# PeterFWS/Structure-PLP-SLAM

Measured on NVIDIA H100. Metric: frames_per_sec_extract_match_poseopt, higher is better.
Workload: dtype u8/f64

## Files before the change

structure-plp-slam_b200/csrc/orb.cu:

```cuda
#include "common.cuh"
#include <cuda.h>
#include <stdlib.h>
#include "brief_pattern.inc"
#include "quadtree_kernels.cuh"

namespace plp {

namespace {

constexpr int kMaxLevels = 16;
constexpr int kHalfPatch = 15;
constexpr int kCellSize = 64;
constexpr int kOverlap = 6;

struct LevelInfo {
    int w, h, pitch;
    size_t offset;
    size_t blur_offset;
    int cells_x, cells_y;
    int cell_base;
    int num_cells;
    int budget;
    int slot_base;
    int slot_cap;
    float scale_factor;
    float size;
};

struct CellDesc {
    short level, i, j, pad;
    short min_x, min_y, max_x, max_y;
};

struct BlurTile {
    short level, x0, y0, pad;
};

struct OrbDev {
    int num_levels, rows, cols;
    int num_cells;
    int total_slots;
    int out_cap;
    int ini_thr, min_thr;
    LevelInfo lv[kMaxLevels];
    int u_max[16];
    const uint8_t *img0;
    size_t img0_step, img0_frame_stride;
    const uint8_t *mask;
    size_t mask_step;
    uint8_t *pyr;
    size_t pyr_frame_bytes;
    uint8_t *blur;
    size_t blur_frame_bytes;
    const BlurTile *blur_tiles;
    int num_blur_tiles;
    const CellDesc *cells;
    uint32_t *cell_buf;
    int *cell_cnt;
    LevelKp *lvl_kp;
    int *lvl_cnt;
    uint8_t *qt_scratch;
    size_t qt_scratch_per_job;
    int *status;
};

__device__ __forceinline__ const uint8_t *level_ptr(const OrbDev &P, int b, int l) {
    return l == 0 ? P.img0 + (size_t)b * P.img0_frame_stride : P.pyr + (size_t)b * P.pyr_frame_bytes + P.lv[l].offset;
}
__device__ __forceinline__ int level_pitch(const OrbDev &P, int l) { return l == 0 ? (int)P.img0_step : P.lv[l].pitch; }

constexpr int kBtW = 64, kBtH = 32;
constexpr int kBoxW = 96, kBoxH = kBtH + 6, kBoxX = 16;
static_assert(kBoxW >= kBoxX + kBtW + 3 && kBoxW % 16 == 0 && kBoxX % 16 == 0 && kBtW % 16 == 0,
              "TMA box: 16-byte aligned start and extent covering the 3-pixel halo");
static_assert(kBoxH % 2 == 0 && kBtH % 2 == 0, "the blur passes work on pairs of rows");
constexpr int kBoxStage = (kBoxH * kBoxW + 127) & ~127;
constexpr int kTilePitch = kBoxW;
constexpr int kTileRows = kCellSize + kOverlap;

struct BlurMaps {
    CUtensorMap m[kMaxLevels];
};

__device__ __forceinline__ uint32_t smem_u32(const void *p) { return (uint32_t)__cvta_generic_to_shared(p); }

__device__ __forceinline__ void mbar_init(uint32_t bar) { asm volatile("mbarrier.init.shared::cta.b64 [%0], 1;" ::"r"(bar)); }

__device__ __forceinline__ bool mbar_wait(uint32_t bar, uint32_t parity) {
    uint32_t done = 0;
    for (int spin = 0; spin < (1 << 14) && !done; ++spin)
        asm volatile(
// ... 3 lines not shown
            : "memory");
    return done != 0;
}

__device__ __forceinline__ void mbar_expect_tx(uint32_t bar, uint32_t bytes) {
    asm volatile("mbarrier.arrive.expect_tx.shared::cta.b64 _, [%0], %1;" ::"r"(bar), "r"(bytes) : "memory");
}

__device__ __forceinline__ void tma_box_load(uint32_t dst, const CUtensorMap *tm, int x, int y, int f, uint32_t bar) {
    asm volatile(
        "cp.async.bulk.tensor.3d.shared::cluster.global.mbarrier::complete_tx::bytes [%0], [%1, {%2, %3, %4}], [%5];"
        ::"r"(dst), "l"(tm), "r"(x), "r"(y), "r"(f), "r"(bar)
        : "memory");
}

constexpr int kResizeRows = 8;
__global__ void __launch_bounds__(256) pyr_resize_kernel(OrbDev P, int l, const short4 *__restrict__ xtab,
                                                         const short4 *__restrict__ ytab) {
    const int b = blockIdx.y;
    const int dw = P.lv[l].w, dh = P.lv[l].h, dpitch = P.lv[l].pitch;
    const int quads = (dw + 3) >> 2, strips = (dh + kResizeRows - 1) / kResizeRows;
    const int q = blockIdx.x * blockDim.x + threadIdx.x;
    if (q >= quads * strips) return;
    const int strip = q / quads, x0 = (q - strip * quads) * 4;
    const uint8_t *src = level_ptr(P, b, l - 1);
    const int spitch = level_pitch(P, l - 1);
    uint8_t *dst = const_cast<uint8_t *>(level_ptr(P, b, l));
    int sx0[4], sx1[4], a0[4], a1[4];
#pragma unroll
    for (int k = 0; k < 4; ++k) {
        const short4 xt = xtab[min(x0 + k, dw - 1)];
        sx0[k] = xt.x;
        sx1[k] = xt.y;
        a0[k] = xt.z;
        a1[k] = xt.w;
    }
    const int y_end = min(dh, (strip + 1) * kResizeRows);
    for (int y = strip * kResizeRows; y < y_end; ++y) {
        const short4 yt = ytab[y];
        const uint8_t *S0 = src + (size_t)yt.x * spitch, *S1 = src + (size_t)yt.y * spitch;
        const int b0 = yt.z, b1 = yt.w;
        uint32_t packed = 0;
#pragma unroll
        for (int k = 0; k < 4; ++k) {
            const int r0 = S0[sx0[k]] * a0[k] + S0[sx1[k]] * a1[k];
            const int r1 = S1[sx0[k]] * a0[k] + S1[sx1[k]] * a1[k];
            const int v = (((b0 * (r0 >> 4)) >> 16) + ((b1 * (r1 >> 4)) >> 16) + 2) >> 2;
            packed |= (uint32_t)(v & 0xff) << (8 * k);
        }
        *reinterpret_cast<uint32_t *>(dst + (size_t)y * dpitch + x0) = packed;
    }
}

__device__ __forceinline__ uint32_t fast_m_pair(const uint8_t *pa, const uint8_t *pb) {
    const uint32_t v2 = ((uint32_t)pa[0] + 256u) | (((uint32_t)pb[0] + 256u) << 16);
    uint32_t d[16];
#define PLP_RING(k, off) d[k] = v2 - ((uint32_t)pa[off] | ((uint32_t)pb[off] << 16))
    PLP_RING(0, 3 * kTilePitch);
    PLP_RING(1, 3 * kTilePitch + 1);
    PLP_RING(2, 2 * kTilePitch + 2);
    PLP_RING(3, 1 * kTilePitch + 3);
    PLP_RING(4, 3);
    PLP_RING(5, -1 * kTilePitch + 3);
    PLP_RING(6, -2 * kTilePitch + 2);
    PLP_RING(7, -3 * kTilePitch + 1);
// ... 296 lines not shown
    }
    __syncthreads();
    if (n > 0) fast_cell_emit(P, b, first + n - 1, S);
}

constexpr int kDescWarps = 4;
constexpr int kDescRun = 8;
constexpr int kDescMinBlocks = 5;
constexpr int kDiscRows = 2 * kHalfPatch + 1, kDiscPitch = 48;
constexpr int kWinHalf = 18, kWinRows = 2 * kWinHalf + 1, kWinPitch = 64;
constexpr int kDiscBytes = kDiscRows * kDiscPitch;
constexpr int kDescStage = kDiscBytes + kWinRows * kWinPitch;
static_assert(kDiscBytes % 16 == 0 && kDescStage % 16 == 0, "16-byte copies into every row of the ring");
static_assert(15 + kDiscRows <= kDiscPitch && 15 + kWinRows <= kWinPitch, "the aligned supersets fit the rows");

__device__ __forceinline__ int reflect101(int p, int len) {
    if (p < 0) p = -p;
    if (p >= len) p = 2 * (len - 1) - p;
    return p;
}

__device__ __forceinline__ float fast_atan2_deg(float y, float x) {
    const float scale = (float)(180.0 / 3.14159265358979323846);
    const float p1 = 0.9997878412794807f * scale, p3 = -0.3258083974640975f * scale,
                p5 = 0.1555786518463281f * scale, p7 = -0.04432655554792128f * scale;
    const float ax = fabsf(x), ay = fabsf(y);
    float a, c, c2;
    if (ax >= ay) {
        c = __fdiv_rn(ay, ax + (float)2.2204460492503131e-16);
        c2 = c * c;
        a = (((p7 * c2 + p5) * c2 + p3) * c2 + p1) * c;
    } else {
        c = __fdiv_rn(ax, ay + (float)2.2204460492503131e-16);
        c2 = c * c;
        a = 90.f - (((p7 * c2 + p5) * c2 + p3) * c2 + p1) * c;
    }
// ... 8 lines not shown
    return c1 + v2 * (c2 + c3 * v2);
}
__device__ __forceinline__ float util_cos(float v) {
    const float PI = 3.14159265358979f, PI_2 = PI / 2.0f, TWO_PI = 2.0f * PI, INV_TWO_PI = 1.0f / TWO_PI,
                THREE_PI_2 = 3.0f * PI_2;
    v = v - (float)cv_floor((double)(v * INV_TWO_PI)) * TWO_PI;
    v = (0.0f < v) ? v : -v;
    if (v < PI_2) return poly_cos(v);
    if (v < PI) return -poly_cos(PI - v);
    if (v < THREE_PI_2) return -poly_cos(v - PI);
    return poly_cos(TWO_PI - v);
}
__device__ __forceinline__ float util_sin(float v) {
    const float PI_2 = 3.14159265358979f / 2.0f;
    return util_cos(PI_2 - v);
}


__device__ __forceinline__ void blur_row4(const uint32_t *w, uint32_t h[4]) {
    const uint32_t A = w[0], B = w[1], C = w[2];
    const uint32_t kW1 = 0x38302212u, kW2 = 0x00122230u;
    h[0] = __dp4a(__funnelshift_r(A, B, 8), kW1, __dp4a(__funnelshift_r(B, C, 8), kW2, 0u));
    h[1] = __dp4a(__funnelshift_r(A, B, 16), kW1, __dp4a(__funnelshift_r(B, C, 16), kW2, 0u));
    h[2] = __dp4a(__funnelshift_r(A, B, 24), kW1, __dp4a(__funnelshift_r(B, C, 24), kW2, 0u));
    h[3] = __dp4a(B, kW1, __dp4a(C, kW2, 0u));
}
__device__ __forceinline__ void blur_h_pass(const uint8_t *box, uint32_t *h2) {
    const uint32_t *src32 = reinterpret_cast<const uint32_t *>(box);
    for (int i = threadIdx.x; i < (kBoxH / 2) * (kBtW / 4); i += blockDim.x) {
        const int rp = i / (kBtW / 4), j = i % (kBtW / 4);
        const uint32_t *w = src32 + 2 * rp * (kBoxW / 4) + j + (kBoxX - 4) / 4;
        uint32_t e[4], o[4];
        blur_row4(w, e);
        blur_row4(w + kBoxW / 4, o);
        *reinterpret_cast<uint4 *>(h2 + rp * kBtW + 4 * j) =
            make_uint4(__byte_perm(e[0], o[0], 0x5410), __byte_perm(e[1], o[1], 0x5410), __byte_perm(e[2], o[2], 0x5410),
                       __byte_perm(e[3], o[3], 0x5410));
    }
}

constexpr int kBlurThreads = 256;
static_assert((kBtH / 2) * (kBtW / 4) == kBlurThreads, "one vertical-pass job per thread");
__device__ __forceinline__ void blur_v_pass(const uint32_t *h2, uint8_t *dst, int dpitch, int x0, int y0, int W, int H) {
    const int q = threadIdx.x / (kBtW / 4), px = (threadIdx.x % (kBtW / 4)) * 4;
    const int y = y0 + 2 * q;
    if (y >= H || x0 + px >= W) return;
    uint32_t r[4][4];
#pragma unroll
    for (int k = 0; k < 4; ++k) {
        const uint4 v = *reinterpret_cast<const uint4 *>(h2 + (q + k) * kBtW + px);
        r[k][0] = v.x;
        r[k][1] = v.y;
        r[k][2] = v.z;
        r[k][3] = v.w;
    }
    auto row = [&](uint32_t k0, uint32_t k1, uint32_t k2, uint32_t k3) -> uint32_t {
        uint32_t a[4];
#pragma unroll
        for (int c = 0; c < 4; ++c)
            a[c] = __dp2a_lo(r[0][c], k0, __dp2a_lo(r[1][c], k1, __dp2a_lo(r[2][c], k2, __dp2a_lo(r[3][c], k3, 32768u))));
        return __byte_perm(__byte_perm(a[0], a[1], 0x0062), __byte_perm(a[2], a[3], 0x0062), 0x5410);
    };
    uint8_t *d = dst + (size_t)y * dpitch + x0 + px;
    *reinterpret_cast<uint32_t *>(d) = row(0x2212u, 0x3830u, 0x2230u, 0x0012u);
    if (y + 1 < H) *reinterpret_cast<uint32_t *>(d + dpitch) = row(0x1200u, 0x3022u, 0x3038u, 0x1222u);
}

__global__ void __launch_bounds__(kBlurThreads) blur_tiles_kernel(OrbDev P) {
    __shared__ __align__(16) uint8_t s_src[kBoxH * kBoxW];
    __shared__ __align__(16) uint32_t s_h2[(kBoxH / 2) * kBtW];
    const int b = blockIdx.y, tid = threadIdx.x;
    const BlurTile t = P.blur_tiles[blockIdx.x];
    const int l = t.level, W = P.lv[l].w, H = P.lv[l].h;
    const uint8_t *img = level_ptr(P, b, l);
    const int pitch = level_pitch(P, l);
    constexpr int kCols = kBtW + 8;
    for (int i = tid; i < kBoxH * kCols; i += kBlurThreads) {
        const int py = i / kCols, px = i - py * kCols;
        const int gy = reflect101(min(t.y0 - 3 + py, H + 2), H);
        const int gx = reflect101(min(max(t.x0 - 4 + px, -3), W + 2), W);
        s_src[py * kBoxW + kBoxX - 4 + px] = img[(size_t)gy * pitch + gx];
    }
    __syncthreads();
    blur_h_pass(s_src, s_h2);
    __syncthreads();
    blur_v_pass(s_h2, P.blur + (size_t)b * P.blur_frame_bytes + P.lv[l].blur_offset, P.lv[l].pitch, t.x0, t.y0, W, H);
}

__device__ void blur_reflect_box(uint8_t *box, int bx0, int by0, int W, int H) {
    for (int i = threadIdx.x; i < kBoxH * 6; i += blockDim.x) {
        const int py = i / 6, k = i - py * 6;
        const int gx = k < 3 ? k - 3 : W + (k - 3), gy = by0 + py;
        const int px = gx - bx0;
        if (gy < 0 || gy >= H || px < 0 || px >= kBoxW) continue;
        box[py * kBoxW + px] = box[py * kBoxW + (reflect101(gx, W) - bx0)];
    }
    __syncthreads();
    for (int i = threadIdx.x; i < 6 * kBoxW; i += blockDim.x) {
        const int k = i / kBoxW, px = i - k * kBoxW;
        const int gy = k < 3 ? k - 3 : H + (k - 3);
        const int py = gy - by0;
        if (py < 0 || py >= kBoxH) continue;
        box[py * kBoxW + px] = box[(reflect101(gy, H) - by0) * kBoxW + px];
    }
    __syncthreads();
}

constexpr int kBlurRun = 4;
__global__ void __launch_bounds__(kBlurThreads) blur_tiles_tma_kernel(const __grid_constant__ BlurMaps M, OrbDev P, int run) {
    __shared__ __align__(128) uint8_t s_src[2][kBoxStage];
    __shared__ __align__(16) uint32_t s_h2[(kBoxH / 2) * kBtW];
    __shared__ __align__(8) unsigned long long s_bar[2];
    const int b = blockIdx.y, tid = threadIdx.x;
    const int first = blockIdx.x * run, n = min(run, P.num_blur_tiles - first);
    if (tid == 0) {
        mbar_init(smem_u32(&s_bar[0]));
        mbar_init(smem_u32(&s_bar[1]));
        asm volatile("fence.mbarrier_init.release.cluster;" ::: "memory");
    }
    __syncthreads();
    auto issue = [&](int i) {
        const BlurTile t = P.blur_tiles[first + i];
        const uint32_t bar = smem_u32(&s_bar[i & 1]);
        mbar_expect_tx(bar, kBoxH * kBoxW);
        tma_box_load(smem_u32(s_src[i & 1]), &M.m[t.level], t.x0 - kBoxX, t.y0 - 3, b, bar);
    };
    if (tid == 0) issue(0);
    for (int i = 0; i < n; ++i) {
        __syncthreads();
        if (tid == 0 && i + 1 < n) {
            asm volatile("fence.proxy.async.shared::cta;" ::: "memory");
            issue(i + 1);
        }
        const BlurTile t = P.blur_tiles[first + i];
        const int l = t.level, W = P.lv[l].w, H = P.lv[l].h;
        const int bx0 = t.x0 - kBoxX, by0 = t.y0 - 3;
        uint8_t *box = s_src[i & 1];
        if (!mbar_wait(smem_u32(&s_bar[i & 1]), (i >> 1) & 1)) P.status[b] = 3;
        if (t.x0 < 3 || by0 < 0 || t.x0 + kBtW + 3 > W || by0 + kBoxH > H) blur_reflect_box(box, bx0, by0, W, H);
        blur_h_pass(box, s_h2);
        __syncthreads();
        blur_v_pass(s_h2, P.blur + (size_t)b * P.blur_frame_bytes + P.lv[l].blur_offset, P.lv[l].pitch, t.x0, t.y0, W, H);
    }
}

__device__ __forceinline__ void cp_async16(void *dst, const void *src) {
    asm volatile("cp.async.ca.shared.global [%0], [%1], 16;" ::"r"(smem_u32(dst)), "l"(src) : "memory");
}
__device__ __forceinline__ void cp_async_commit() { asm volatile("cp.async.commit_group;" ::: "memory"); }
__device__ __forceinline__ void cp_async_wait_prev() { asm volatile("cp.async.wait_group 1;" ::: "memory"); }

__device__ __forceinline__ int dp4a_us(uint32_t a, uint32_t b, int c) {
    int d;
    asm("dp4a.u32.s32 %0, %1, %2, %3;" : "=r"(d) : "r"(a), "r"(b), "r"(c));
    return d;
}

template <int J>
// ... 197 lines not shown
    J.scratch_per_job = D.qt_scratch_per_job;
    J.status = D.status;
    return J;
}

struct plp_orb {
    plp_ctx *ctx = nullptr;
    plp_orb_params params;
    int rows = 0, cols = 0, max_batch = 0;
    OrbDev dev;
    std::vector<float> scale_factors, inv_scale_factors, level_sigma_sq, inv_level_sigma_sq;
    std::vector<uint32_t> num_keypts_per_level;
    std::vector<CellDesc> cells;
    short4 *d_xtab[kMaxLevels] = {nullptr};
    short4 *d_ytab[kMaxLevels] = {nullptr};
    CellDesc *d_cells = nullptr;
    uint8_t *d_pyr = nullptr;
    uint8_t *d_blur = nullptr;
    BlurTile *d_blur_tiles = nullptr;
    std::vector<BlurTile> blur_tiles;
    uint8_t *d_img = nullptr;
    uint8_t *d_mask = nullptr;
    uint32_t *d_cell_buf = nullptr;
    int *d_cell_cnt = nullptr;
    LevelKp *d_lvl_kp = nullptr;
    int *d_lvl_cnt = nullptr;
    uint8_t *d_qt_scratch = nullptr;
    int *d_status = nullptr;
    plp_keypoint *d_kp = nullptr;
    uint8_t *d_desc = nullptr;
// ... 22 lines not shown
            return nullptr;
        return (EncodeTiledFn)p;
    }();
    return fn;
}
static bool encode_level_map(CUtensorMap *m, const uint8_t *base, int w, int h, int frames, size_t pitch, size_t frame_stride) {
    EncodeTiledFn enc = tensor_map_encoder();
    if (!enc || ((uintptr_t)base & 15) || (pitch & 15) || (frame_stride & 15) || w < 1 || h < 1 || frames < 1) return false;
    const cuuint64_t dims[3] = {(cuuint64_t)w, (cuuint64_t)h, (cuuint64_t)frames};
    const cuuint64_t strides[2] = {(cuuint64_t)pitch, (cuuint64_t)frame_stride};
    const cuuint32_t box[3] = {(cuuint32_t)kBoxW, (cuuint32_t)kBoxH, 1u}, estr[3] = {1u, 1u, 1u};
    return enc(m, CU_TENSOR_MAP_DATA_TYPE_UINT8, 3, (void *)base, dims, strides, box, estr, CU_TENSOR_MAP_INTERLEAVE_NONE,
               CU_TENSOR_MAP_SWIZZLE_NONE, CU_TENSOR_MAP_L2_PROMOTION_L2_128B, CU_TENSOR_MAP_FLOAT_OOB_FILL_NONE) == CUDA_SUCCESS;
}


static void build_resize_tables(int sw, int sh, int dw, int dh, std::vector<short4> &xt, std::vector<short4> &yt) {
    const double inv_scale_x = (double)dw / sw, inv_scale_y = (double)dh / sh;
    const double scale_x = 1. / inv_scale_x, scale_y = 1. / inv_scale_y;
    xt.resize(dw);
    yt.resize(dh);
    for (int dx = 0; dx < dw; ++dx) {
        float fx = (float)((dx + 0.5) * scale_x - 0.5);
        int sx = cv_floor(fx);
        fx -= sx;
        if (sx < 0) {
            fx = 0;
            sx = 0;
        }
        if (sx >= sw - 1) {
            fx = 0;
            sx = sw - 1;
        }
        short4 t;
        t.x = (short)sx;
        t.y = (short)std::min(sx + 1, sw - 1);
        t.z = (short)lrintf((1.f - fx) * 2048);
        t.w = (short)lrintf(fx * 2048);
        xt[dx] = t;
    }
    for (int dy = 0; dy < dh; ++dy) {
        float fy = (float)((dy + 0.5) * scale_y - 0.5);
        int sy = cv_floor(fy);
        fy -= sy;
        short4 t;
        t.x = (short)std::min(std::max(sy, 0), sh - 1);
        t.y = (short)std::min(std::max(sy + 1, 0), sh - 1);
        t.z = (short)lrintf((1.f - fy) * 2048);
        t.w = (short)lrintf(fy * 2048);
        yt[dy] = t;
    }
}

extern "C" {

void plp_orb_destroy(plp_orb *o) {
    if (!o) return;
    cudaSetDevice(o->ctx->device);
    cudaStreamSynchronize(o->ctx->stream);
    for (int l = 0; l < kMaxLevels; ++l) {
        if (o->d_xtab[l]) cudaFree(o->d_xtab[l]);
        if (o->d_ytab[l]) cudaFree(o->d_ytab[l]);
    }
    void *ptrs[] = {o->d_blur, o->d_blur_tiles, o->d_cells, o->d_pyr, o->d_img, o->d_mask, o->d_cell_buf, o->d_cell_cnt, o->d_lvl_kp,
                    o->d_lvl_cnt, o->d_qt_scratch, o->d_status, o->d_kp, o->d_desc, o->d_n};
    for (void *p : ptrs)
        if (p) cudaFree(p);
// ... 73 lines not shown
        if (l == 0) {
            V.w = cols;
            V.h = rows;
        } else {
            const double scale = o->scale_factors[l];
            V.w = (int)std::round(cols * 1.0 / scale);
            V.h = (int)std::round(rows * 1.0 / scale);
        }
        V.pitch = (V.w + 63) & ~63;
        V.offset = pyr_bytes;
        if (l > 0) pyr_bytes += (size_t)V.pitch * V.h + 256;
        pyr_bytes = (pyr_bytes + 255) & ~(size_t)255;
        V.blur_offset = blur_bytes;
        blur_bytes += (size_t)V.pitch * V.h + 256;
        blur_bytes = (blur_bytes + 255) & ~(size_t)255;
        for (int y0 = 0; y0 < V.h; y0 += kBtH)
            for (int x0 = 0; x0 < V.w; x0 += kBtW) o->blur_tiles.push_back(BlurTile{(short)l, (short)x0, (short)y0, 0});
        V.budget = (int)o->num_keypts_per_level[l];
        V.scale_factor = o->scale_factors[l];
        V.size = (float)(unsigned)(31 * o->scale_factors[l]);
        V.slot_base = slot_base;
        {
            int g0 = 1;
            if (V.w > 2 * kPatchRadius && V.h > 2 * kPatchRadius) {
                const double ratio = (double)(V.w - 2 * kPatchRadius) / (V.h - 2 * kPatchRadius);
                g0 = ratio > 1 ? (int)std::round(ratio) : (int)std::round(1 / ratio);
            }
            V.slot_cap = 4 * std::max(V.budget, g0) + 8;
        }
        slot_base += V.slot_cap;
        V.cell_base = cell_base;
        V.num_cells = 0;
// ... 37 lines not shown
        qt_max_cells = std::max(qt_max_cells, V.num_cells);
    }
    if (st == PLP_OK && qt_max_cells + 1 > 2 * (qt_max_slots <= kNodeCapSmall ? kNodeCapSmall : kNodeCap)) {
        set_error("orb: a pyramid level of %d FAST cells exceeds the quadtree's cell capacity", qt_max_cells);
        st = PLP_ERR_CAPACITY;
    }
    if (st != PLP_OK) {
        delete o;
        return st;
    }
    D.num_cells = cell_base;
    D.total_slots = slot_base;
    D.out_cap = slot_base;
    D.pyr_frame_bytes = pyr_bytes ? pyr_bytes : 256;
    D.blur_frame_bytes = blur_bytes ? blur_bytes : 256;
    D.num_blur_tiles = (int)o->blur_tiles.size();
    const size_t B = (size_t)max_batch;
#define ORB_ALLOC(ptr, bytes)                                              \
    do {                                                                   \
        cudaError_t e_ = cudaMalloc((void **)&(ptr), (bytes) ? (bytes) : 256); \
        if (e_ != cudaSuccess) {                                           \
            set_error("orb: cudaMalloc(%zu) failed: %s", (size_t)(bytes), cudaGetErrorString(e_)); \
            plp_orb_destroy(o);                                            \
            return PLP_ERR_CUDA;                                           \
        }                                                                  \
    } while (0)
    for (unsigned l = 1; l < L; ++l) {
        std::vector<short4> xt, yt;
        build_resize_tables(D.lv[l - 1].w, D.lv[l - 1].h, D.lv[l].w, D.lv[l].h, xt, yt);
        ORB_ALLOC(o->d_xtab[l], xt.size() * sizeof(short4));
        ORB_ALLOC(o->d_ytab[l], yt.size() * sizeof(short4));
        cudaMemcpy(o->d_xtab[l], xt.data(), xt.size() * sizeof(short4), cudaMemcpyHostToDevice);
        cudaMemcpy(o->d_ytab[l], yt.data(), yt.size() * sizeof(short4), cudaMemcpyHostToDevice);
    }
    ORB_ALLOC(o->d_cells, o->cells.size() * sizeof(CellDesc));
    if (!o->cells.empty())
        cudaMemcpy(o->d_cells, o->cells.data(), o->cells.size() * sizeof(CellDesc), cudaMemcpyHostToDevice);
    ORB_ALLOC(o->d_pyr, B * D.pyr_frame_bytes);
    ORB_ALLOC(o->d_blur, B * D.blur_frame_bytes);
    ORB_ALLOC(o->d_blur_tiles, o->blur_tiles.size() * sizeof(BlurTile));
    if (!o->blur_tiles.empty())
        cudaMemcpy(o->d_blur_tiles, o->blur_tiles.data(), o->blur_tiles.size() * sizeof(BlurTile), cudaMemcpyHostToDevice);
    ORB_ALLOC(o->d_img, B * (size_t)rows * cols);
    ORB_ALLOC(o->d_mask, (size_t)rows * cols);
// ... 56 lines not shown

static plp_status orb_run(plp_orb *o, const uint8_t *d_imgs, int batch, size_t step, const uint8_t *d_mask,
                          size_t mask_step, plp_keypoint *d_kp, uint8_t *d_desc, int32_t *d_n, int32_t *d_status) {
    plp_ctx *ctx = o->ctx;
    OrbDev D = o->dev;
    D.img0 = d_imgs;
    D.img0_step = step;
    D.img0_frame_stride = step * (size_t)o->rows;
    D.mask = d_mask;
    D.mask_step = mask_step;
    D.status = d_status ? d_status : o->d_status;
    o->last_batch = batch;
    o->last_img0 = d_imgs;
    o->last_step = step;
    PLP_CUDA_TRY(cudaMemsetAsync(D.status, 0, (size_t)batch * sizeof(int), ctx->stream));
    for (int l = 1; l < D.num_levels; ++l) {
        const int quads = ((D.lv[l].w + 3) >> 2) * ((D.lv[l].h + kResizeRows - 1) / kResizeRows);
        if (quads <= 0) continue;
        dim3 grid(div_up(quads, 256), batch);
        PLP_LAUNCH(ctx, pyr_resize_kernel, grid, 256, 0, D, l, o->d_xtab[l], o->d_ytab[l]);
    }
    bool tma = o->maps_ok;
    if (tma && (o->map0_img != d_imgs || o->map0_step != step || o->map0_batch != batch)) {
        tma = encode_level_map(&o->maps.m[0], d_imgs, D.lv[0].w, D.lv[0].h, batch, step, D.img0_frame_stride);
        o->map0_img = tma ? d_imgs : nullptr;
        o->map0_step = step;
        o->map0_batch = batch;
    }
    if (D.num_cells > 0) {
        dim3 grid(D.num_cells, batch), grid_run(div_up(D.num_cells, kFastRun), batch);
        if (tma)
            PLP_LAUNCH(ctx, fast_cells_tma_kernel, grid_run, 256, 0, o->maps, D, kFastRun);
        else
            PLP_LAUNCH(ctx, fast_cells_kernel_v2, grid, 256, 0, D);
    }
    if (D.num_blur_tiles > 0) {
        dim3 grid(D.num_blur_tiles, batch), grid_run(div_up(D.num_blur_tiles, kBlurRun), batch);
        if (tma)
            PLP_LAUNCH(ctx, blur_tiles_tma_kernel, grid_run, kBlurThreads, 0, o->maps, D, kBlurRun);
        else
            PLP_LAUNCH(ctx, blur_tiles_kernel, grid, kBlurThreads, 0, D);
    }
    {
        dim3 grid(D.num_levels, batch);
        if (ctx->timing) plp::timing_begin(ctx, o->qt_small ? "quadtree_kernel<1024>" : "quadtree_kernel<2048>");
        const QtJob J = qt_job(D);
        if (o->qt_small)
            kQtSmall<<<grid, kQtThreadsSmall, o->qt_smem, ctx->stream>>>(J);
        else
            kQtLarge<<<grid, kQtThreadsLarge, o->qt_smem, ctx->stream>>>(J);
        if (ctx->timing) plp::timing_end(ctx);
        ctx->launches++;
    }
    {
        const int kp_est = std::max(256, (int)o->params.max_num_keypts);
        dim3 grid(div_up(std::min(D.total_slots, kp_est), kDescWarps * kDescRun), batch);
// ... 132 lines not shown
```

Before: 93160.

## Fuse pyramid resize into per-level blur tile kernel using TMA-loaded boxes

Removes the standalone pyramid resize kernels and computes each next pyramid level from the shared-memory source box already loaded for blurring, launching blur+resize per level in sequence. This avoids re-reading each level from global memory for the resize and removes separate launches. In exchange, levels must be processed serially (blur of level l produces level l+1 before its blur), adding dependency chains and host-side validation that bilinear taps fit within tile boxes.

```diff
diff --git a/structure-plp-slam_b200/csrc/orb.cu b/structure-plp-slam_b200/csrc/orb.cu
--- a/structure-plp-slam_b200/csrc/orb.cu
+++ b/structure-plp-slam_b200/csrc/orb.cu
@@ -3,6 +3,7 @@
 #include <stdlib.h>
 #include "brief_pattern.inc"
 #include "quadtree_kernels.cuh"
+#include "pyramid_kernels.cuh"
 
 namespace plp {
 
@@ -20,6 +21,8 @@
     int cells_x, cells_y;
     int cell_base;
     int num_cells;
+    int tile_base;
+    int num_tiles;
     int budget;
     int slot_base;
     int slot_cap;
@@ -30,10 +33,6 @@
 struct CellDesc {
     short level, i, j, pad;
     short min_x, min_y, max_x, max_y;
-};
-
-struct BlurTile {
-    short level, x0, y0, pad;
 };
 
 struct OrbDev {
@@ -53,7 +52,6 @@
     uint8_t *blur;
     size_t blur_frame_bytes;
     const BlurTile *blur_tiles;
-    int num_blur_tiles;
     const CellDesc *cells;
     uint32_t *cell_buf;
     int *cell_cnt;
@@ -69,12 +67,6 @@
 }
 __device__ __forceinline__ int level_pitch(const OrbDev &P, int l) { return l == 0 ? (int)P.img0_step : P.lv[l].pitch; }
 
-constexpr int kBtW = 64, kBtH = 32;
-constexpr int kBoxW = 96, kBoxH = kBtH + 6, kBoxX = 16;
-static_assert(kBoxW >= kBoxX + kBtW + 3 && kBoxW % 16 == 0 && kBoxX % 16 == 0 && kBtW % 16 == 0,
-              "TMA box: 16-byte aligned start and extent covering the 3-pixel halo");
-static_assert(kBoxH % 2 == 0 && kBtH % 2 == 0, "the blur passes work on pairs of rows");
-constexpr int kBoxStage = (kBoxH * kBoxW + 127) & ~127;
 constexpr int kTilePitch = kBoxW;
 constexpr int kTileRows = kCellSize + kOverlap;
 
@@ -108,41 +100,43 @@
         : "memory");
 }
 
-constexpr int kResizeRows = 8;
-__global__ void __launch_bounds__(256) pyr_resize_kernel(OrbDev P, int l, const short4 *__restrict__ xtab,
-                                                         const short4 *__restrict__ ytab) {
-    const int b = blockIdx.y;
-    const int dw = P.lv[l].w, dh = P.lv[l].h, dpitch = P.lv[l].pitch;
-    const int quads = (dw + 3) >> 2, strips = (dh + kResizeRows - 1) / kResizeRows;
-    const int q = blockIdx.x * blockDim.x + threadIdx.x;
-    if (q >= quads * strips) return;
-    const int strip = q / quads, x0 = (q - strip * quads) * 4;
-    const uint8_t *src = level_ptr(P, b, l - 1);
-    const int spitch = level_pitch(P, l - 1);
-    uint8_t *dst = const_cast<uint8_t *>(level_ptr(P, b, l));
-    int sx0[4], sx1[4], a0[4], a1[4];
-#pragma unroll
-    for (int k = 0; k < 4; ++k) {
-        const short4 xt = xtab[min(x0 + k, dw - 1)];
-        sx0[k] = xt.x;
-        sx1[k] = xt.y;
-        a0[k] = xt.z;
-        a1[k] = xt.w;
-    }
-    const int y_end = min(dh, (strip + 1) * kResizeRows);
-    for (int y = strip * kResizeRows; y < y_end; ++y) {
-        const short4 yt = ytab[y];
-        const uint8_t *S0 = src + (size_t)yt.x * spitch, *S1 = src + (size_t)yt.y * spitch;
-        const int b0 = yt.z, b1 = yt.w;
-        uint32_t packed = 0;
-#pragma unroll
-        for (int k = 0; k < 4; ++k) {
-            const int r0 = S0[sx0[k]] * a0[k] + S0[sx1[k]] * a1[k];
-            const int r1 = S1[sx0[k]] * a0[k] + S1[sx1[k]] * a1[k];
-            const int v = (((b0 * (r0 >> 4)) >> 16) + ((b1 * (r1 >> 4)) >> 16) + 2) >> 2;
-            packed |= (uint32_t)(v & 0xff) << (8 * k);
-        }
-        *reinterpret_cast<uint32_t *>(dst + (size_t)y * dpitch + x0) = packed;
+constexpr int kBlurRun = 4;
+constexpr int kBlurMinBlocks = 8;
+__global__ void __launch_bounds__(kBlurThreads, kBlurMinBlocks) blur_tiles_tma_kernel(const __grid_constant__ BlurMaps M, PyrJob J, int run) {
+    __shared__ __align__(128) uint8_t s_src[2][kBoxStage];
+    __shared__ __align__(16) uint32_t s_h2[(kBoxH / 2) * kBtW];
+    __shared__ __align__(8) unsigned long long s_bar[2];
+    const int b = blockIdx.y, tid = threadIdx.x;
+    const int first = blockIdx.x * run, n = min(run, J.num_tiles - first);
+    const int W = J.w, H = J.h;
+    if (tid == 0) {
+        mbar_init(smem_u32(&s_bar[0]));
+        mbar_init(smem_u32(&s_bar[1]));
+        asm volatile("fence.mbarrier_init.release.cluster;" ::: "memory");
+    }
+    __syncthreads();
+    auto issue = [&](int i) {
+        const BlurTile t = J.tiles[first + i];
+        const uint32_t bar = smem_u32(&s_bar[i & 1]);
+        mbar_expect_tx(bar, kBoxH * kBoxW);
+        tma_box_load(smem_u32(s_src[i & 1]), &M.m[t.level], t.x0 - kBoxX, t.y0 - 3, b, bar);
+    };
+    if (tid == 0) issue(0);
+    for (int i = 0; i < n; ++i) {
+        __syncthreads();
+        if (tid == 0 && i + 1 < n) {
+            asm volatile("fence.proxy.async.shared::cta;" ::: "memory");
+            issue(i + 1);
+        }
+        const BlurTile t = J.tiles[first + i];
+        const int bx0 = t.x0 - kBoxX, by0 = t.y0 - 3;
+        uint8_t *box = s_src[i & 1];
+        if (!mbar_wait(smem_u32(&s_bar[i & 1]), (i >> 1) & 1)) J.status[b] = 3;
+        if (t.x0 < 3 || by0 < 0 || t.x0 + kBtW + 3 > W || by0 + kBoxH > H) blur_reflect_box(box, bx0, by0, W, H);
+        blur_h_pass(box, s_h2);
+        if (J.dst) pyr_resize_tile(box, bx0, by0, t, J, b);
+        __syncthreads();
+        blur_v_pass(s_h2, J.blur + (size_t)b * J.blur_frame, J.blur_pitch, t.x0, t.y0, W, H);
     }
 }
 
@@ -469,12 +463,6 @@
 static_assert(kDiscBytes % 16 == 0 && kDescStage % 16 == 0, "16-byte copies into every row of the ring");
 static_assert(15 + kDiscRows <= kDiscPitch && 15 + kWinRows <= kWinPitch, "the aligned supersets fit the rows");
 
-__device__ __forceinline__ int reflect101(int p, int len) {
-    if (p < 0) p = -p;
-    if (p >= len) p = 2 * (len - 1) - p;
-    return p;
-}
-
 __device__ __forceinline__ float fast_atan2_deg(float y, float x) {
     const float scale = (float)(180.0 / 3.14159265358979323846);
     const float p1 = 0.9997878412794807f * scale, p3 = -0.3258083974640975f * scale,
@@ -513,134 +501,6 @@
 __device__ __forceinline__ float util_sin(float v) {
     const float PI_2 = 3.14159265358979f / 2.0f;
     return util_cos(PI_2 - v);
-}
-
-
-__device__ __forceinline__ void blur_row4(const uint32_t *w, uint32_t h[4]) {
-    const uint32_t A = w[0], B = w[1], C = w[2];
-    const uint32_t kW1 = 0x38302212u, kW2 = 0x00122230u;
-    h[0] = __dp4a(__funnelshift_r(A, B, 8), kW1, __dp4a(__funnelshift_r(B, C, 8), kW2, 0u));
-    h[1] = __dp4a(__funnelshift_r(A, B, 16), kW1, __dp4a(__funnelshift_r(B, C, 16), kW2, 0u));
-    h[2] = __dp4a(__funnelshift_r(A, B, 24), kW1, __dp4a(__funnelshift_r(B, C, 24), kW2, 0u));
-    h[3] = __dp4a(B, kW1, __dp4a(C, kW2, 0u));
-}
-__device__ __forceinline__ void blur_h_pass(const uint8_t *box, uint32_t *h2) {
-    const uint32_t *src32 = reinterpret_cast<const uint32_t *>(box);
-    for (int i = threadIdx.x; i < (kBoxH / 2) * (kBtW / 4); i += blockDim.x) {
-        const int rp = i / (kBtW / 4), j = i % (kBtW / 4);
-        const uint32_t *w = src32 + 2 * rp * (kBoxW / 4) + j + (kBoxX - 4) / 4;
-        uint32_t e[4], o[4];
-        blur_row4(w, e);
-        blur_row4(w + kBoxW / 4, o);
-        *reinterpret_cast<uint4 *>(h2 + rp * kBtW + 4 * j) =
-            make_uint4(__byte_perm(e[0], o[0], 0x5410), __byte_perm(e[1], o[1], 0x5410), __byte_perm(e[2], o[2], 0x5410),
-                       __byte_perm(e[3], o[3], 0x5410));
-    }
-}
-
-constexpr int kBlurThreads = 256;
-static_assert((kBtH / 2) * (kBtW / 4) == kBlurThreads, "one vertical-pass job per thread");
-__device__ __forceinline__ void blur_v_pass(const uint32_t *h2, uint8_t *dst, int dpitch, int x0, int y0, int W, int H) {
-    const int q = threadIdx.x / (kBtW / 4), px = (threadIdx.x % (kBtW / 4)) * 4;
-    const int y = y0 + 2 * q;
-    if (y >= H || x0 + px >= W) return;
-    uint32_t r[4][4];
-#pragma unroll
-    for (int k = 0; k < 4; ++k) {
-        const uint4 v = *reinterpret_cast<const uint4 *>(h2 + (q + k) * kBtW + px);
-        r[k][0] = v.x;
-        r[k][1] = v.y;
-        r[k][2] = v.z;
-        r[k][3] = v.w;
-    }
-    auto row = [&](uint32_t k0, uint32_t k1, uint32_t k2, uint32_t k3) -> uint32_t {
-        uint32_t a[4];
-#pragma unroll
-        for (int c = 0; c < 4; ++c)
-            a[c] = __dp2a_lo(r[0][c], k0, __dp2a_lo(r[1][c], k1, __dp2a_lo(r[2][c], k2, __dp2a_lo(r[3][c], k3, 32768u))));
-        return __byte_perm(__byte_perm(a[0], a[1], 0x0062), __byte_perm(a[2], a[3], 0x0062), 0x5410);
-    };
-    uint8_t *d = dst + (size_t)y * dpitch + x0 + px;
-    *reinterpret_cast<uint32_t *>(d) = row(0x2212u, 0x3830u, 0x2230u, 0x0012u);
-    if (y + 1 < H) *reinterpret_cast<uint32_t *>(d + dpitch) = row(0x1200u, 0x3022u, 0x3038u, 0x1222u);
-}
-
-__global__ void __launch_bounds__(kBlurThreads) blur_tiles_kernel(OrbDev P) {
-    __shared__ __align__(16) uint8_t s_src[kBoxH * kBoxW];
-    __shared__ __align__(16) uint32_t s_h2[(kBoxH / 2) * kBtW];
-    const int b = blockIdx.y, tid = threadIdx.x;
-    const BlurTile t = P.blur_tiles[blockIdx.x];
-    const int l = t.level, W = P.lv[l].w, H = P.lv[l].h;
-    const uint8_t *img = level_ptr(P, b, l);
-    const int pitch = level_pitch(P, l);
-    constexpr int kCols = kBtW + 8;
-    for (int i = tid; i < kBoxH * kCols; i += kBlurThreads) {
-        const int py = i / kCols, px = i - py * kCols;
-        const int gy = reflect101(min(t.y0 - 3 + py, H + 2), H);
-        const int gx = reflect101(min(max(t.x0 - 4 + px, -3), W + 2), W);
-        s_src[py * kBoxW + kBoxX - 4 + px] = img[(size_t)gy * pitch + gx];
-    }
-    __syncthreads();
-    blur_h_pass(s_src, s_h2);
-    __syncthreads();
-    blur_v_pass(s_h2, P.blur + (size_t)b * P.blur_frame_bytes + P.lv[l].blur_offset, P.lv[l].pitch, t.x0, t.y0, W, H);
-}
-
-__device__ void blur_reflect_box(uint8_t *box, int bx0, int by0, int W, int H) {
-    for (int i = threadIdx.x; i < kBoxH * 6; i += blockDim.x) {
-        const int py = i / 6, k = i - py * 6;
-        const int gx = k < 3 ? k - 3 : W + (k - 3), gy = by0 + py;
-        const int px = gx - bx0;
-        if (gy < 0 || gy >= H || px < 0 || px >= kBoxW) continue;
-        box[py * kBoxW + px] = box[py * kBoxW + (reflect101(gx, W) - bx0)];
-    }
-    __syncthreads();
-    for (int i = threadIdx.x; i < 6 * kBoxW; i += blockDim.x) {
-        const int k = i / kBoxW, px = i - k * kBoxW;
-        const int gy = k < 3 ? k - 3 : H + (k - 3);
-        const int py = gy - by0;
-        if (py < 0 || py >= kBoxH) continue;
-        box[py * kBoxW + px] = box[(reflect101(gy, H) - by0) * kBoxW + px];
-    }
-    __syncthreads();
-}
-
-constexpr int kBlurRun = 4;
-__global__ void __launch_bounds__(kBlurThreads) blur_tiles_tma_kernel(const __grid_constant__ BlurMaps M, OrbDev P, int run) {
-    __shared__ __align__(128) uint8_t s_src[2][kBoxStage];
-    __shared__ __align__(16) uint32_t s_h2[(kBoxH / 2) * kBtW];
-    __shared__ __align__(8) unsigned long long s_bar[2];
-    const int b = blockIdx.y, tid = threadIdx.x;
-    const int first = blockIdx.x * run, n = min(run, P.num_blur_tiles - first);
-    if (tid == 0) {
-        mbar_init(smem_u32(&s_bar[0]));
-        mbar_init(smem_u32(&s_bar[1]));
-        asm volatile("fence.mbarrier_init.release.cluster;" ::: "memory");
-    }
-    __syncthreads();
-    auto issue = [&](int i) {
-        const BlurTile t = P.blur_tiles[first + i];
-        const uint32_t bar = smem_u32(&s_bar[i & 1]);
-        mbar_expect_tx(bar, kBoxH * kBoxW);
-        tma_box_load(smem_u32(s_src[i & 1]), &M.m[t.level], t.x0 - kBoxX, t.y0 - 3, b, bar);
-    };
-    if (tid == 0) issue(0);
-    for (int i = 0; i < n; ++i) {
-        __syncthreads();
-        if (tid == 0 && i + 1 < n) {
-            asm volatile("fence.proxy.async.shared::cta;" ::: "memory");
-            issue(i + 1);
-        }
-        const BlurTile t = P.blur_tiles[first + i];
-        const int l = t.level, W = P.lv[l].w, H = P.lv[l].h;
-        const int bx0 = t.x0 - kBoxX, by0 = t.y0 - 3;
-        uint8_t *box = s_src[i & 1];
-        if (!mbar_wait(smem_u32(&s_bar[i & 1]), (i >> 1) & 1)) P.status[b] = 3;
-        if (t.x0 < 3 || by0 < 0 || t.x0 + kBtW + 3 > W || by0 + kBoxH > H) blur_reflect_box(box, bx0, by0, W, H);
-        blur_h_pass(box, s_h2);
-        __syncthreads();
-        blur_v_pass(s_h2, P.blur + (size_t)b * P.blur_frame_bytes + P.lv[l].blur_offset, P.lv[l].pitch, t.x0, t.y0, W, H);
-    }
 }
 
 __device__ __forceinline__ void cp_async16(void *dst, const void *src) {
@@ -868,6 +728,7 @@
     std::vector<CellDesc> cells;
     short4 *d_xtab[kMaxLevels] = {nullptr};
     short4 *d_ytab[kMaxLevels] = {nullptr};
+    int tap_words[kMaxLevels] = {0};
     CellDesc *d_cells = nullptr;
     uint8_t *d_pyr = nullptr;
     uint8_t *d_blur = nullptr;
@@ -920,43 +781,6 @@
                CU_TENSOR_MAP_SWIZZLE_NONE, CU_TENSOR_MAP_L2_PROMOTION_L2_128B, CU_TENSOR_MAP_FLOAT_OOB_FILL_NONE) == CUDA_SUCCESS;
 }
 
-
-static void build_resize_tables(int sw, int sh, int dw, int dh, std::vector<short4> &xt, std::vector<short4> &yt) {
-    const double inv_scale_x = (double)dw / sw, inv_scale_y = (double)dh / sh;
-    const double scale_x = 1. / inv_scale_x, scale_y = 1. / inv_scale_y;
-    xt.resize(dw);
-    yt.resize(dh);
-    for (int dx = 0; dx < dw; ++dx) {
-        float fx = (float)((dx + 0.5) * scale_x - 0.5);
-        int sx = cv_floor(fx);
-        fx -= sx;
-        if (sx < 0) {
-            fx = 0;
-            sx = 0;
-        }
-        if (sx >= sw - 1) {
-            fx = 0;
-            sx = sw - 1;
-        }
-        short4 t;
-        t.x = (short)sx;
-        t.y = (short)std::min(sx + 1, sw - 1);
-        t.z = (short)lrintf((1.f - fx) * 2048);
-        t.w = (short)lrintf(fx * 2048);
-        xt[dx] = t;
-    }
-    for (int dy = 0; dy < dh; ++dy) {
-        float fy = (float)((dy + 0.5) * scale_y - 0.5);
-        int sy = cv_floor(fy);
-        fy -= sy;
-        short4 t;
-        t.x = (short)std::min(std::max(sy, 0), sh - 1);
-        t.y = (short)std::min(std::max(sy + 1, 0), sh - 1);
-        t.z = (short)lrintf((1.f - fy) * 2048);
-        t.w = (short)lrintf(fy * 2048);
-        yt[dy] = t;
-    }
-}
 
 extern "C" {
 
@@ -1060,8 +884,6 @@
         V.blur_offset = blur_bytes;
         blur_bytes += (size_t)V.pitch * V.h + 256;
         blur_bytes = (blur_bytes + 255) & ~(size_t)255;
-        for (int y0 = 0; y0 < V.h; y0 += kBtH)
-            for (int x0 = 0; x0 < V.w; x0 += kBtW) o->blur_tiles.push_back(BlurTile{(short)l, (short)x0, (short)y0, 0});
         V.budget = (int)o->num_keypts_per_level[l];
         V.scale_factor = o->scale_factors[l];
         V.size = (float)(unsigned)(31 * o->scale_factors[l]);
@@ -1129,7 +951,26 @@
     D.out_cap = slot_base;
     D.pyr_frame_bytes = pyr_bytes ? pyr_bytes : 256;
     D.blur_frame_bytes = blur_bytes ? blur_bytes : 256;
-    D.num_blur_tiles = (int)o->blur_tiles.size();
+    std::vector<std::vector<short4>> xtabs(L), ytabs(L);
+    for (unsigned l = 1; l < L; ++l) {
+        build_resize_tables(D.lv[l - 1].w, D.lv[l - 1].h, D.lv[l].w, D.lv[l].h, xtabs[l], ytabs[l]);
+        o->tap_words[l] = pyr_taps_in_words(xtabs[l].data(), D.lv[l].w);
+    }
+    for (unsigned l = 0; l < L; ++l) {
+        LevelInfo &V = D.lv[l];
+        const bool next = l + 1 < L;
+        const short4 *xt = next ? xtabs[l + 1].data() : nullptr, *yt = next ? ytabs[l + 1].data() : nullptr;
+        const int dw = next ? D.lv[l + 1].w : 0, dh = next ? D.lv[l + 1].h : 0;
+        V.tile_base = (int)o->blur_tiles.size();
+        pyr_level_tiles((int)l, V.w, V.h, xt, yt, dw, dh, o->blur_tiles);
+        V.num_tiles = (int)o->blur_tiles.size() - V.tile_base;
+        if (next && !pyr_tiles_fit(o->blur_tiles.data() + V.tile_base, V.num_tiles, xt, yt, dw)) {
+            set_error("orb: scale factor %g: a bilinear tap of level %u lies outside the source box of its blur tile",
+                      (double)params->scale_factor, l + 1);
+            delete o;
+            return PLP_ERR_INVALID;
+        }
+    }
     const size_t B = (size_t)max_batch;
 #define ORB_ALLOC(ptr, bytes)                                              \
     do {                                                                   \
@@ -1141,8 +982,7 @@
         }                                                                  \
     } while (0)
     for (unsigned l = 1; l < L; ++l) {
-        std::vector<short4> xt, yt;
-        build_resize_tables(D.lv[l - 1].w, D.lv[l - 1].h, D.lv[l].w, D.lv[l].h, xt, yt);
+        const std::vector<short4> &xt = xtabs[l], &yt = ytabs[l];
         ORB_ALLOC(o->d_xtab[l], xt.size() * sizeof(short4));
         ORB_ALLOC(o->d_ytab[l], yt.size() * sizeof(short4));
         cudaMemcpy(o->d_xtab[l], xt.data(), xt.size() * sizeof(short4), cudaMemcpyHostToDevice);
@@ -1229,12 +1069,6 @@
     o->last_img0 = d_imgs;
     o->last_step = step;
     PLP_CUDA_TRY(cudaMemsetAsync(D.status, 0, (size_t)batch * sizeof(int), ctx->stream));
-    for (int l = 1; l < D.num_levels; ++l) {
-        const int quads = ((D.lv[l].w + 3) >> 2) * ((D.lv[l].h + kResizeRows - 1) / kResizeRows);
-        if (quads <= 0) continue;
-        dim3 grid(div_up(quads, 256), batch);
-        PLP_LAUNCH(ctx, pyr_resize_kernel, grid, 256, 0, D, l, o->d_xtab[l], o->d_ytab[l]);
-    }
     bool tma = o->maps_ok;
     if (tma && (o->map0_img != d_imgs || o->map0_step != step || o->map0_batch != batch)) {
         tma = encode_level_map(&o->maps.m[0], d_imgs, D.lv[0].w, D.lv[0].h, batch, step, D.img0_frame_stride);
@@ -1242,19 +1076,41 @@
         o->map0_step = step;
         o->map0_batch = batch;
     }
+    for (int l = 0; l < D.num_levels; ++l) {
+        const LevelInfo &V = D.lv[l];
+        if (V.num_tiles == 0) continue;
+        const bool next = l + 1 < D.num_levels;
+        PyrJob J;
+        J.src = l == 0 ? D.img0 : D.pyr + V.offset;
+        J.src_step = l == 0 ? D.img0_step : (size_t)V.pitch;
+        J.src_frame = l == 0 ? D.img0_frame_stride : D.pyr_frame_bytes;
+        J.w = V.w;
+        J.h = V.h;
+        J.blur = D.blur + V.blur_offset;
+        J.blur_frame = D.blur_frame_bytes;
+        J.blur_pitch = V.pitch;
+        J.dst = next ? D.pyr + D.lv[l + 1].offset : nullptr;
+        J.dst_frame = D.pyr_frame_bytes;
+        J.dst_pitch = next ? D.lv[l + 1].pitch : 0;
+        J.dw = next ? D.lv[l + 1].w : 0;
+        J.xtab = next ? o->d_xtab[l + 1] : nullptr;
+        J.ytab = next ? o->d_ytab[l + 1] : nullptr;
+        J.tap_words = next ? o->tap_words[l + 1] : 0;
+        J.tiles = D.blur_tiles + V.tile_base;
+        J.num_tiles = V.num_tiles;
+        J.status = D.status;
+        if (tma)
+            PLP_LAUNCH(ctx, blur_tiles_tma_kernel, dim3(div_up(V.num_tiles, kBlurRun), batch), kBlurThreads, 0, o->maps, J,
+                       kBlurRun);
+        else
+            PLP_LAUNCH(ctx, blur_tiles_kernel, dim3(V.num_tiles, batch), kBlurThreads, 0, J);
+    }
     if (D.num_cells > 0) {
         dim3 grid(D.num_cells, batch), grid_run(div_up(D.num_cells, kFastRun), batch);
         if (tma)
             PLP_LAUNCH(ctx, fast_cells_tma_kernel, grid_run, 256, 0, o->maps, D, kFastRun);
         else
             PLP_LAUNCH(ctx, fast_cells_kernel_v2, grid, 256, 0, D);
-    }
-    if (D.num_blur_tiles > 0) {
-        dim3 grid(D.num_blur_tiles, batch), grid_run(div_up(D.num_blur_tiles, kBlurRun), batch);
-        if (tma)
-            PLP_LAUNCH(ctx, blur_tiles_tma_kernel, grid_run, kBlurThreads, 0, o->maps, D, kBlurRun);
-        else
-            PLP_LAUNCH(ctx, blur_tiles_kernel, grid, kBlurThreads, 0, D);
     }
     {
         dim3 grid(D.num_levels, batch);
diff --git a/structure-plp-slam_b200/csrc/pyramid_kernels.cuh b/structure-plp-slam_b200/csrc/pyramid_kernels.cuh
--- /dev/null
+++ b/structure-plp-slam_b200/csrc/pyramid_kernels.cuh
@@ -0,0 +1,285 @@
+#pragma once
+#include <math.h>
+#include <stddef.h>
+#include <stdint.h>
+
+#include <vector>
+
+#include "devmath.cuh"
+
+namespace plp {
+
+namespace {
+
+constexpr int kBtW = 64, kBtH = 32;
+constexpr int kBoxW = 96, kBoxH = kBtH + 6, kBoxX = 16;
+constexpr int kPlainCol0 = kBoxX - 4;
+static_assert(kBoxW >= kBoxX + kBtW + 3 && kBoxW % 16 == 0 && kBoxX % 16 == 0 && kBtW % 16 == 0,
+              "TMA box: 16-byte aligned start and extent covering the 3-pixel halo");
+static_assert(kBoxH % 2 == 0 && kBtH % 2 == 0, "the blur passes work on pairs of rows");
+constexpr int kBoxStage = (kBoxH * kBoxW + 127) & ~127;
+constexpr int kBlurThreads = 256;
+static_assert((kBtH / 2) * (kBtW / 4) == kBlurThreads, "one vertical-pass job per thread");
+
+struct BlurTile {
+    short level, x0, y0, pad;
+    short q0, nq, r0, nr;
+};
+
+struct PyrJob {
+    const uint8_t *src;
+    size_t src_step, src_frame;
+    int w, h;
+    uint8_t *blur;
+    size_t blur_frame;
+    int blur_pitch;
+    uint8_t *dst;
+    size_t dst_frame;
+    int dst_pitch, dw;
+    const short4 *xtab, *ytab;
+    int tap_words;
+    const BlurTile *tiles;
+    int num_tiles;
+    int *status;
+};
+
+__device__ __forceinline__ int reflect101(int p, int len) {
+    if (p < 0) p = -p;
+    if (p >= len) p = 2 * (len - 1) - p;
+    return p;
+}
+
+constexpr int kResizeLanes = 16;
+__device__ __forceinline__ void pyr_resize_tile(const uint8_t *box, int bx0, int by0, const BlurTile &t, const PyrJob &J,
+                                                int b) {
+    uint8_t *dst = J.dst + (size_t)b * J.dst_frame + (size_t)t.r0 * J.dst_pitch;
+    const uint8_t *rows = box - by0 * kBoxW - bx0;
+    const int ri0 = threadIdx.x / kResizeLanes, rstep = blockDim.x / kResizeLanes;
+    for (int qi = threadIdx.x % kResizeLanes; qi < t.nq; qi += kResizeLanes) {
+        const int x = (t.q0 + qi) * 4;
+        int c0[4], c1[4];
+        uint32_t w[4];
+#pragma unroll
+        for (int k = 0; k < 4; ++k) {
+            const short4 xt = J.xtab[min(x + k, J.dw - 1)];
+            c0[k] = xt.x;
+            c1[k] = xt.y;
+            w[k] = (uint32_t)(uint16_t)xt.z | (uint32_t)xt.w << 16;
+        }
+        if (J.tap_words) {
+            const int cb = c0[0] & ~3;
+            const uint32_t sh = (uint32_t)(c0[0] & 3) * 8;
+            uint32_t sel = 0;
+#pragma unroll
+            for (int k = 0; k < 4; ++k) sel |= ((uint32_t)(c0[k] - c0[0]) | (uint32_t)(c1[k] - c0[0]) << 4) << (8 * k);
+            for (int r = ri0; r < t.nr; r += rstep) {
+                const short4 yt = J.ytab[t.r0 + r];
+                const uint32_t *s0 = reinterpret_cast<const uint32_t *>(rows + yt.x * kBoxW + cb);
+                const uint32_t *s1 = reinterpret_cast<const uint32_t *>(rows + yt.y * kBoxW + cb);
+                const uint32_t u0 = s0[1], u1 = s1[1];
+                const uint32_t A0 = __funnelshift_r(s0[0], u0, sh), B0 = __funnelshift_r(u0, s0[2], sh);
+                const uint32_t A1 = __funnelshift_r(s1[0], u1, sh), B1 = __funnelshift_r(u1, s1[2], sh);
+                const uint32_t b0 = (uint32_t)yt.z << 16, b1 = (uint32_t)yt.w << 16;
+                uint32_t packed = 0;
+#pragma unroll
+                for (int k = 0; k < 4; ++k) {
+                    const uint32_t h0 = __dp2a_lo(w[k], __byte_perm(A0, B0, sel >> (8 * k)), 0u);
+                    const uint32_t h1 = __dp2a_lo(w[k], __byte_perm(A1, B1, sel >> (8 * k)), 0u);
+                    packed |= ((__umulhi(b0, h0 >> 4) + __umulhi(b1, h1 >> 4) + 2) >> 2) << (8 * k);
+                }
+                *reinterpret_cast<uint32_t *>(dst + (size_t)r * J.dst_pitch + x) = packed;
+            }
+        } else {
+            for (int r = ri0; r < t.nr; r += rstep) {
+                const short4 yt = J.ytab[t.r0 + r];
+                const uint8_t *s0 = rows + yt.x * kBoxW, *s1 = rows + yt.y * kBoxW;
+                const uint32_t b0 = (uint32_t)yt.z << 16, b1 = (uint32_t)yt.w << 16;
+                uint32_t packed = 0;
+#pragma unroll
+                for (int k = 0; k < 4; ++k) {
+                    const uint32_t h0 = __dp2a_lo(w[k], (uint32_t)s0[c0[k]] | (uint32_t)s0[c1[k]] << 8, 0u);
+                    const uint32_t h1 = __dp2a_lo(w[k], (uint32_t)s1[c0[k]] | (uint32_t)s1[c1[k]] << 8, 0u);
+                    packed |= ((__umulhi(b0, h0 >> 4) + __umulhi(b1, h1 >> 4) + 2) >> 2) << (8 * k);
+                }
+                *reinterpret_cast<uint32_t *>(dst + (size_t)r * J.dst_pitch + x) = packed;
+            }
+        }
+    }
+}
+
+
+__device__ __forceinline__ void blur_row4(const uint32_t *w, uint32_t h[4]) {
+    const uint32_t A = w[0], B = w[1], C = w[2];
+    const uint32_t kW1 = 0x38302212u, kW2 = 0x00122230u;
+    h[0] = __dp4a(__funnelshift_r(A, B, 8), kW1, __dp4a(__funnelshift_r(B, C, 8), kW2, 0u));
+    h[1] = __dp4a(__funnelshift_r(A, B, 16), kW1, __dp4a(__funnelshift_r(B, C, 16), kW2, 0u));
+    h[2] = __dp4a(__funnelshift_r(A, B, 24), kW1, __dp4a(__funnelshift_r(B, C, 24), kW2, 0u));
+    h[3] = __dp4a(B, kW1, __dp4a(C, kW2, 0u));
+}
+__device__ __forceinline__ void blur_h_pass(const uint8_t *box, uint32_t *h2) {
+    const uint32_t *src32 = reinterpret_cast<const uint32_t *>(box);
+    for (int i = threadIdx.x; i < (kBoxH / 2) * (kBtW / 4); i += blockDim.x) {
+        const int rp = i / (kBtW / 4), j = i % (kBtW / 4);
+        const uint32_t *w = src32 + 2 * rp * (kBoxW / 4) + j + (kBoxX - 4) / 4;
+        uint32_t e[4], o[4];
+        blur_row4(w, e);
+        blur_row4(w + kBoxW / 4, o);
+        *reinterpret_cast<uint4 *>(h2 + rp * kBtW + 4 * j) =
+            make_uint4(__byte_perm(e[0], o[0], 0x5410), __byte_perm(e[1], o[1], 0x5410), __byte_perm(e[2], o[2], 0x5410),
+                       __byte_perm(e[3], o[3], 0x5410));
+    }
+}
+
+__device__ __forceinline__ void blur_v_pass(const uint32_t *h2, uint8_t *dst, int dpitch, int x0, int y0, int W, int H) {
+    const int q = threadIdx.x / (kBtW / 4), px = (threadIdx.x % (kBtW / 4)) * 4;
+    const int y = y0 + 2 * q;
+    if (y >= H || x0 + px >= W) return;
+    uint32_t r[4][4];
+#pragma unroll
+    for (int k = 0; k < 4; ++k) {
+        const uint4 v = *reinterpret_cast<const uint4 *>(h2 + (q + k) * kBtW + px);
+        r[k][0] = v.x;
+        r[k][1] = v.y;
+        r[k][2] = v.z;
+        r[k][3] = v.w;
+    }
+    auto row = [&](uint32_t k0, uint32_t k1, uint32_t k2, uint32_t k3) -> uint32_t {
+        uint32_t a[4];
+#pragma unroll
+        for (int c = 0; c < 4; ++c)
+            a[c] = __dp2a_lo(r[0][c], k0, __dp2a_lo(r[1][c], k1, __dp2a_lo(r[2][c], k2, __dp2a_lo(r[3][c], k3, 32768u))));
+        return __byte_perm(__byte_perm(a[0], a[1], 0x0062), __byte_perm(a[2], a[3], 0x0062), 0x5410);
+    };
+    uint8_t *d = dst + (size_t)y * dpitch + x0 + px;
+    *reinterpret_cast<uint32_t *>(d) = row(0x2212u, 0x3830u, 0x2230u, 0x0012u);
+    if (y + 1 < H) *reinterpret_cast<uint32_t *>(d + dpitch) = row(0x1200u, 0x3022u, 0x3038u, 0x1222u);
+}
+
+__device__ __forceinline__ void blur_reflect_box(uint8_t *box, int bx0, int by0, int W, int H) {
+    for (int i = threadIdx.x; i < kBoxH * 6; i += blockDim.x) {
+        const int py = i / 6, k = i - py * 6;
+        const int gx = k < 3 ? k - 3 : W + (k - 3), gy = by0 + py;
+        const int px = gx - bx0;
+        if (gy < 0 || gy >= H || px < 0 || px >= kBoxW) continue;
+        box[py * kBoxW + px] = box[py * kBoxW + (reflect101(gx, W) - bx0)];
+    }
+    __syncthreads();
+    for (int i = threadIdx.x; i < 6 * kBoxW; i += blockDim.x) {
+        const int k = i / kBoxW, px = i - k * kBoxW;
+        const int gy = k < 3 ? k - 3 : H + (k - 3);
+        const int py = gy - by0;
+        if (py < 0 || py >= kBoxH) continue;
+        box[py * kBoxW + px] = box[(reflect101(gy, H) - by0) * kBoxW + px];
+    }
+    __syncthreads();
+}
+
+__global__ void __launch_bounds__(kBlurThreads) blur_tiles_kernel(PyrJob J) {
+    __shared__ __align__(16) uint8_t s_src[kBoxH * kBoxW];
+    __shared__ __align__(16) uint32_t s_h2[(kBoxH / 2) * kBtW];
+    const int b = blockIdx.y, tid = threadIdx.x;
+    const BlurTile t = J.tiles[blockIdx.x];
+    const int W = J.w, H = J.h;
+    const uint8_t *img = J.src + (size_t)b * J.src_frame;
+    constexpr int kCols = kBoxW - kPlainCol0;
+    for (int i = tid; i < kBoxH * kCols; i += kBlurThreads) {
+        const int py = i / kCols, px = i - py * kCols;
+        const int gy = reflect101(min(t.y0 - 3 + py, H + 2), H);
+        const int gx = reflect101(min(max(t.x0 - 4 + px, -3), W + 2), W);
+        s_src[py * kBoxW + kPlainCol0 + px] = img[(size_t)gy * J.src_step + gx];
+    }
+    __syncthreads();
+    blur_h_pass(s_src, s_h2);
+    if (J.dst) pyr_resize_tile(s_src, t.x0 - kBoxX, t.y0 - 3, t, J, b);
+    __syncthreads();
+    blur_v_pass(s_h2, J.blur + (size_t)b * J.blur_frame, J.blur_pitch, t.x0, t.y0, W, H);
+}
+
+
+inline void build_resize_tables(int sw, int sh, int dw, int dh, std::vector<short4> &xt, std::vector<short4> &yt) {
+    const double inv_scale_x = (double)dw / sw, inv_scale_y = (double)dh / sh;
+    const double scale_x = 1. / inv_scale_x, scale_y = 1. / inv_scale_y;
+    xt.resize(dw);
+    yt.resize(dh);
+    for (int dx = 0; dx < dw; ++dx) {
+        float fx = (float)((dx + 0.5) * scale_x - 0.5);
+        int sx = cv_floor(fx);
+        fx -= sx;
+        if (sx < 0) {
+            fx = 0;
+            sx = 0;
+        }
+        if (sx >= sw - 1) {
+            fx = 0;
+            sx = sw - 1;
+        }
+        short4 t;
+        t.x = (short)sx;
+        t.y = (short)(sx + 1 < sw - 1 ? sx + 1 : sw - 1);
+        t.z = (short)lrintf((1.f - fx) * 2048);
+        t.w = (short)lrintf(fx * 2048);
+        xt[dx] = t;
+    }
+    for (int dy = 0; dy < dh; ++dy) {
+        float fy = (float)((dy + 0.5) * scale_y - 0.5);
+        int sy = cv_floor(fy);
+        fy -= sy;
+        const int s0 = sy < 0 ? 0 : sy, s1 = sy + 1 < 0 ? 0 : sy + 1;
+        short4 t;
+        t.x = (short)(s0 < sh - 1 ? s0 : sh - 1);
+        t.y = (short)(s1 < sh - 1 ? s1 : sh - 1);
+        t.z = (short)lrintf((1.f - fy) * 2048);
+        t.w = (short)lrintf(fy * 2048);
+        yt[dy] = t;
+    }
+}
+
+inline void pyr_level_tiles(int l, int w, int h, const short4 *xt, const short4 *yt, int dw, int dh, std::vector<BlurTile> &out) {
+    for (int y0 = 0; y0 < h; y0 += kBtH)
+        for (int x0 = 0; x0 < w; x0 += kBtW) {
+            BlurTile t{(short)l, (short)x0, (short)y0, 0, 0, 0, 0, 0};
+            if (xt) {
+                int q0 = 0, q1 = 0, r0 = 0, r1 = 0;
+                const int nq = (dw + 3) / 4;
+                while (q0 < nq && xt[4 * q0].x < x0) ++q0;
+                for (q1 = q0; q1 < nq && xt[4 * q1].x < x0 + kBtW; ++q1) {
+                }
+                while (r0 < dh && yt[r0].x < y0) ++r0;
+                for (r1 = r0; r1 < dh && yt[r1].x < y0 + kBtH; ++r1) {
+                }
+                if (q1 > q0 && r1 > r0) {
+                    t.q0 = (short)q0;
+                    t.nq = (short)(q1 - q0);
+                    t.r0 = (short)r0;
+                    t.nr = (short)(r1 - r0);
+                }
+            }
+            out.push_back(t);
+        }
+}
+
+inline bool pyr_taps_in_words(const short4 *xt, int dw) {
+    for (int x = 0; x < dw; ++x)
+        if (xt[x].y - xt[x & ~3].x > 7) return false;
+    return true;
+}
+
+inline bool pyr_tiles_fit(const BlurTile *tiles, int n, const short4 *xt, const short4 *yt, int dw) {
+    for (int i = 0; i < n; ++i) {
+        const BlurTile &t = tiles[i];
+        if (t.nq == 0) continue;
+        const int xlo = t.x0 - (kBoxX - kPlainCol0), xhi = t.x0 + kBoxW - kBoxX - 1;
+        const int ylo = t.y0 - 3, yhi = t.y0 + kBoxH - 4;
+        for (int x = 4 * t.q0; x < 4 * (t.q0 + t.nq); ++x) {
+            const short4 c = xt[x < dw - 1 ? x : dw - 1];
+            if (c.x < xlo || c.y > xhi || c.y < xlo || c.x > xhi) return false;
+        }
+        for (int y = t.r0; y < t.r0 + t.nr; ++y)
+            if (yt[y].x < ylo || yt[y].y > yhi || yt[y].y < ylo || yt[y].x > yhi) return false;
+    }
+    return true;
+}
+
+}
+
+}
```

After: 94380, median of 6. 1.3% higher.
